# ectucker1/voxel-raytracing

Hardware: AMD Instinct MI355X
Metric: Mrays/sec at 1080p treehouse.vox; achieved HBM GB/s vs MI355X peak (higher is better)
Workload: dtype f32; 1 GPU; synthetic:treehouse(seed=2) 256^3 stand-in for treehouse.vox, 1920x1080, primary rays only (BASELINE configs[1]); 128 frame(s)/step (128 per GPU, consecutive poses, one K1 launch per step), 16-row strips over 1 GPU(s); traversal=AUTO, bytes_out_per_px=37, device=AMD Radeon Graphics (gfx950:sramecc+:xnack-)

## Files before the change

voxel-raytracing_amd/csrc/vrt_api.hip:

```cpp
#include <cstdio>
#include <cstdlib>
#include <cstring>

#include "image_io.h"
#include "vox_reader.h"
#include "vrt_host.h"

using namespace vrt;

static thread_local std::string g_err;

int vrt::fail(int code, const std::string& msg) { g_err = msg; return code; }

struct OptName { const char* name; const char* env; int DevOptions::*field; };
static const OptName kOptNames[] = {
    {"tile_tags", "VRT_TILE_TAGS", &DevOptions::tile_tags}, {"box_rect", "VRT_BOX_RECT", &DevOptions::box_rect},
    {"xcd_regions", "VRT_XCD_REGIONS", &DevOptions::xcd_regions}, {"fast_loop", "VRT_FAST_LOOP", &DevOptions::fast_loop},
    {"no_bounce_kernel", "VRT_NO_BOUNCE_KERNEL", &DevOptions::no_bounce_kernel}, {"sky_fast", "VRT_SKY_FAST", &DevOptions::sky_fast},
    {"sky_span", "VRT_SKY_SPAN", &DevOptions::sky_span},
    {"packed_bounces", "VRT_PACKED_BOUNCES", &DevOptions::packed_bounces}, {"ao_batch", "VRT_AO_BATCH", &DevOptions::ao_batch}, {"tags_async", "VRT_TAGS_ASYNC", &DevOptions::tags_async},
    {"hit_table", "VRT_HIT_TABLE", &DevOptions::hit_table},
    {"thresh_runs", "VRT_THRESH_RUNS", &DevOptions::thresh_runs}, {"segment_budget", "VRT_SEGMENT_BUDGET", &DevOptions::segment_budget}, {"denoise_th16", "VRT_DENOISE_TH", &DevOptions::denoise_th16}, {"denoise_packed", "VRT_DENOISE_PACKED", &DevOptions::denoise_packed},
    {"denoise_pair", "VRT_DENOISE_PAIR", &DevOptions::denoise_pair}, {"denoise_p0", "VRT_DENOISE_P0", &DevOptions::denoise_p0}, {"denoise_pair_wgs", "VRT_DENOISE_PAIR_WGS", &DevOptions::denoise_pair_wgs},
    {"denoise_verified", "VRT_DENOISE_VERIFIED", &DevOptions::denoise_verified}, {"denoise_guard_div8", "VRT_DENOISE_GUARD_DIV8", &DevOptions::denoise_guard_div8},
    {"denoise_count", "VRT_DENOISE_COUNT", &DevOptions::denoise_count},
    {"open_cells", "VRT_OPEN_CELLS", &DevOptions::open_cells}, {"df_prefetch", "VRT_DF_PREFETCH", &DevOptions::df_prefetch},
    {"df_own", "VRT_DF_OWN", &DevOptions::df_own},
};

extern "C" {

const char* vrt_last_error(void) { return g_err.c_str(); }

int vrt_ctx_create(int device, vrt_ctx** out)
{
    if (!out) return fail(VRT_ERR_INVALID, "vrt_ctx_create: out is NULL");
    int n = 0;
    hipError_t e = hipGetDeviceCount(&n);
    if (e != hipSuccess || n <= 0)
        return fail(VRT_ERR_NO_DEVICE, std::string("no HIP device available (") + hipGetErrorString(e) +
                                           "); this library has no CPU fallback");
    if (device < 0 || device >= n) return fail(VRT_ERR_INVALID, "vrt_ctx_create: device index out of range");
    HIPCHK(hipSetDevice(device));
    vrt_ctx* c = new vrt_ctx();
    c->device = device;
    for (const OptName& o : kOptNames) {
        const char* e = getenv(o.env);
        if (e && e[0] >= '0' && e[0] <= '9') c->opt.*(o.field) = atoi(e);
    }
// ... 460 lines not shown
        c->tile_tags[b].reset(); c->tile_tags_words[b] = 0;
        HIPCHK(c->tile_tags[b].alloc((words + 3) * sizeof(uint32_t)));
        HIPCHK(hipMemsetAsync(c->tile_tags[b].get(), 0, (words + 3) * sizeof(uint32_t), c->stream));
        HIPCHK(hipStreamSynchronize(c->stream));
        c->tile_tags_words[b] = words;
        c->tag_read_valid[b] = false;
    }
    if (++c->tile_gen == 0u) {
        HIPCHK(hipStreamSynchronize(c->stream));
        if (c->tag_stream) HIPCHK(hipStreamSynchronize(c->tag_stream));
        for (int q = 0; q < 2; q++)
            if (c->tile_tags[q]) HIPCHK(hipMemsetAsync(c->tile_tags[q].get(), 0, c->tile_tags_words[q] * sizeof(uint32_t), c->stream));
        HIPCHK(hipStreamSynchronize(c->stream));
        c->tile_gen = 1u;
    }
    p.tile_tags = c->tile_tags[b].get(); p.tile_gen = c->tile_gen;
    if (p.fused_shade == 1 && p.table) {
        const size_t bytes = (size_t)vrt::verdict_pitch((uint32_t)(p.tiles_x * (p.tile_w / 8))) * (size_t)(p.tiles_y_local * (p.tile_h / 8)) * (size_t)n;
        if (c->verdict_bytes[b] < bytes) {
            HIPCHK(hipStreamSynchronize(c->stream));
            if (c->tag_stream) HIPCHK(hipStreamSynchronize(c->tag_stream));
            c->verdicts[b].reset(); c->verdict_bytes[b] = 0;
            HIPCHK(c->verdicts[b].alloc(bytes));
            c->verdict_bytes[b] = bytes;
        }
        p.verdicts = c->verdicts[b].get();
    }
    if (!tags) {
        std::vector<uint32_t> ones((size_t)n, c->tile_gen);
        HIPCHK(hipMemcpyAsync(c->tile_tags[b].get(), ones.data(), (size_t)n * 4, hipMemcpyHostToDevice, c->stream));
        HIPCHK(launch_block_verdicts(p, c->stream));
        return VRT_OK;
    }
    p.cells = s->cells.get(); p.n_cells = s->n_cells; p.cell_size = s->bricks ? 8u : 4u;
    const bool async = c->opt.tags_async >= 2 || (c->opt.tags_async != 0 && hipStreamQuery(c->stream) == hipErrorNotReady);
    if (!async) {
        HIPCHK(launch_tile_tags(p, c->stream));
        HIPCHK(launch_block_verdicts(p, c->stream));
        return VRT_OK;
    }
    if (!c->tag_stream) {
        HIPCHK(hipStreamCreateWithFlags(&c->tag_stream, hipStreamNonBlocking));
        for (int q = 0; q < 2; q++) {
            HIPCHK(hipEventCreateWithFlags(&c->tag_done[q], hipEventDisableTiming));
            HIPCHK(hipEventCreateWithFlags(&c->tag_read[q], hipEventDisableTiming));
        }
        HIPCHK(hipEventRecord(c->tag_read[b], c->stream));
        HIPCHK(hipStreamWaitEvent(c->tag_stream, c->tag_read[b], 0));
    }
    if (c->tag_read_valid[b]) HIPCHK(hipStreamWaitEvent(c->tag_stream, c->tag_read[b], 0));
    if (tab >= 0) HIPCHK(hipStreamWaitEvent(c->tag_stream, c->tab_uploaded[tab], 0));
    HIPCHK(launch_tile_tags(p, c->tag_stream));
    HIPCHK(launch_block_verdicts(p, c->tag_stream));
    HIPCHK(hipEventRecord(c->tag_done[b], c->tag_stream));
    HIPCHK(hipStreamWaitEvent(c->stream, c->tag_done[b], 0));
    return VRT_OK;
}

static int render_frames(vrt_ctx* c, const vrt_scene* s, int n, const vrt_push* pushes, const vrt_settings* st,
                         const vrt_frame* frames, const vrt_shard* shards, int per_frame)
{
    const Launch l = {n, pushes, st, frames, shards, per_frame, pushes[0].screen_size[0], pushes[0].screen_size[1]};
    int rc = launch_args(c, s, l);
    if (rc != VRT_OK) return rc;
    const bool counts = count_planes(l);
    const uint8_t* count_fields = nullptr;
    if (counts && !s->bricks && s->open_cells) {
// ... 240 lines not shown
```

voxel-raytracing_amd/csrc/vrt_api_edit.hip:

```cpp
#include <cstddef>
#include <cstring>

#include "vrt_host.h"
#include "vrt_brush_launch.h"
#include "vrt_flood_launch.h"
#include "vrt_voxelize_launch.h"
#include "vrt_morph_launch.h"
#include "vrt_components_launch.h"

using namespace vrt;

static_assert(VRT_BRUSH_BOX == VRT_BRUSH_SHAPE_BOX && VRT_BRUSH_ELLIPSOID == VRT_BRUSH_SHAPE_ELLIPSOID && VRT_BRUSH_CAPSULE == VRT_BRUSH_SHAPE_CAPSULE,
              "include/vrt.h and csrc/vrt_brush.h number the shapes differently");
static_assert(VRT_BRUSH_SET == VRT_BRUSH_MODE_SET && VRT_BRUSH_PAINT == VRT_BRUSH_MODE_PAINT && VRT_BRUSH_ADD == VRT_BRUSH_MODE_ADD &&
              VRT_BRUSH_REPLACE == VRT_BRUSH_MODE_REPLACE, "include/vrt.h and csrc/vrt_brush.h number the modes differently");
static_assert(VRT_FLOOD_SAME == VRT_FLOOD_MATCH_SAME && VRT_FLOOD_SOLID == VRT_FLOOD_MATCH_SOLID && VRT_FLOOD_FACES == VRT_FLOOD_CONN_FACES &&
              VRT_FLOOD_CORNERS == VRT_FLOOD_CONN_CORNERS && VRT_FLOOD_MEASURE == VRT_FLOOD_FLAG_MEASURE,
              "include/vrt.h and csrc/vrt_flood.h number the predicates, connectivities or flags differently");
static_assert(VRT_VOXELIZE_SURFACE == VRT_VOXELIZE_FILL_SURFACE && VRT_VOXELIZE_SOLID == VRT_VOXELIZE_FILL_SOLID,
              "include/vrt.h and csrc/vrt_voxelize.h number the fills differently");
static_assert(VRT_MORPH_DILATE == VRT_MORPH_OP_DILATE && VRT_MORPH_ERODE == VRT_MORPH_OP_ERODE && VRT_MORPH_OPEN == VRT_MORPH_OP_OPEN &&
              VRT_MORPH_CLOSE == VRT_MORPH_OP_CLOSE && VRT_MORPH_HOLLOW == VRT_MORPH_OP_HOLLOW && VRT_MORPH_FACES == VRT_MORPH_CONN_FACES &&
              VRT_MORPH_CORNERS == VRT_MORPH_CONN_CORNERS && VRT_MORPH_BORDER_SOLID == VRT_MORPH_FLAG_BORDER_SOLID && VRT_MORPH_MEASURE == VRT_MORPH_FLAG_MEASURE,
              "include/vrt.h and csrc/vrt_morph.h number the operations, connectivities or flags differently");
// ... 57 lines not shown
    b.nb[0] = d.W / 8; b.nb[1] = d.H / 8; b.nb[2] = d.D / 8;
    b.n = (size_t)b.nb[0] * b.nb[1] * b.nb[2];
    b.npad = ((size_t)b.nb[0] + 2u) * ((size_t)b.nb[1] + 2u) * ((size_t)b.nb[2] + 2u);
    b.cstride = (size_t)d.bcoarse_stride;
    return b;
}

uint64_t brick_scene_bytes(const vrt_scene* s)
{
    const BrickDims b = brick_dims(s);
    return b.npad * 8ull + (uint64_t)s->bcap * 512ull * 9ull + 256 * sizeof(vrt_material) + (uint64_t)s->cells_room * 4ull +
           b.npad * 4ull + b.n + 8ull * b.cstride + s->scratch_bytes();
}

void brick_cell_add(vrt_scene* s, uint32_t slot, uint32_t pc)
{
    s->cell_pos[slot] = (uint32_t)s->hcells.size();
    s->hcells.push_back(brick_cell_code(pc, s->d.vol.pbx, s->d.vol.pby));
    s->cell_slot.push_back(slot);
}

void brick_cell_remove(vrt_scene* s, uint32_t slot)
{
    const uint32_t pos = s->cell_pos[slot], last = (uint32_t)s->hcells.size() - 1u;
    s->hcells[pos] = s->hcells[last]; s->cell_slot[pos] = s->cell_slot[last];
    s->cell_pos[s->cell_slot[pos]] = pos;
    s->hcells.pop_back(); s->cell_slot.pop_back();
    s->cell_pos[slot] = kNoBrick;
}

hipError_t brick_upload_cells(vrt_scene* s)
{
    const size_t n = s->hcells.size();
    s->n_cells = 0; s->cells_ok = false;
    if (n > kMaxCells || n > s->cells_room) return hipSuccess;
    if (n) { const hipError_t e = hipMemcpy(s->cells.get(), s->hcells.data(), n * 4, hipMemcpyHostToDevice); if (e != hipSuccess) return e; }
    s->n_cells = (uint32_t)n; s->cells_ok = true;
    return hipSuccess;
}

hipError_t brick_build_coarse(vrt_ctx* c, vrt_scene* s, uint8_t* tmp0, uint8_t* tmp1, bool pack)
{
    const BrickDims b = brick_dims(s);
    hipError_t e = launch_build_df(s->bocc.get(), b.nb[0], b.nb[1], b.nb[2], s->bcoarse.get(), b.cstride, tmp0, tmp1, c->stream, VRT_BRICK_EDIT_CAP);
    if (e == hipSuccess && s->open_cells) e = launch_open_cells(s->bocc.get(), b.nb[0], b.nb[1], b.nb[2], s->bcoarse.get(), b.cstride, tmp0, tmp1, c->stream, 0x80);
    if (e == hipSuccess && pack) e = launch_brick_pack(s->bgrid.get(), s->bcoarse.get(), b.cstride, b.npad, s->bentry.get(), c->stream);
    return e;
}

int brick_scene_edit(vrt_ctx* c, vrt_scene* s, const EditBox& box, const EditIds& src, const std::string& name)
{
    const VolumeView& d = s->d.vol;
    const BrickDims bd = brick_dims(s);
    BrickEdit e;
    e.nbx = bd.nb[0]; e.nby = bd.nb[1]; e.nbz = bd.nb[2]; e.pbx = d.pbx; e.pby = d.pby;
    EditSpan f[3];
    size_t nT = 1, nF = 1, nbox = 1;
    for (int a = 0; a < 3; a++) {
        e.lo[a] = box.lo[a]; e.hi[a] = box.hi[a];
        const EditSpan t = brick_span_t(box.lo[a], box.hi[a]);
        e.t_lo[a] = t.lo; e.t_n[a] = t.hi - t.lo;
        f[a] = brick_span_f(t, bd.nb[a]);
        nT *= (size_t)e.t_n[a]; nF *= (size_t)(f[a].hi - f[a].lo); nbox *= (size_t)(box.hi[a] - box.lo[a]);
    }
    const bool rule = brick_edit_in_place(e.nbx, e.nby, e.nbz, box.lo, box.hi);
    const bool ids = src.boxed();
    const size_t ids_room = ids ? round256(nbox) : 0, t_room = round256(nT * 4);
    const size_t list_max = rule ? nF : ((size_t)s->n_occ + nT < (size_t)s->bcap ? (size_t)s->n_occ + nT : (size_t)s->bcap);
    const size_t list_room = round256(list_max * 8);
    const size_t coarse_room = rule ? bedit_coarse_scratch_bytes(e, bd.cstride, s->open_cells) : 2 * round256(bd.n);
// ... 799 lines not shown
```

voxel-raytracing_amd/csrc/vrt_api_scene.hip:

```cpp
#include <atomic>
#include <cstdio>
#include <cstring>
#include <memory>

#include "image_io.h"
#include "vox_reader.h"
#include "vox_writer.h"
#include "vrt_host.h"
#define VRT_SCENE_READ_LAUNCHERS
#include "vrt_scene_read.h"

using namespace vrt;

static std::atomic<uint64_t> g_shade_gen{0};

extern "C" {

void vrt_scene_free(vrt_ctx* c, vrt_scene* s)
{
    if (!s) return;
    if (c) { hipSetDevice(c->device); hipStreamSynchronize(c->stream); }
    delete s;
}

// ... 55 lines not shown
    return rc == VRT_OK ? vrt_scene_set_blue_noise(c, s, grey, 1, 1) : rc;
}

void vrt::drop_count_fields(vrt_scene* s)
{
    if (!s->df_counts) return;
    s->df_counts_raw.reset(); s->df_counts = nullptr;
    s->bytes -= s->df_bytes;
}

hipError_t vrt::build_fields(vrt_ctx* c, const vrt_scene* s, uint8_t* dst, bool open)
{
    const VolumeView& d = s->d.vol;
    const size_t nvox = (size_t)d.W * (size_t)d.H * (size_t)d.D, ndf = df_field_bytes(d.W, d.H, d.D);
    hipError_t e = hipMemsetAsync(dst, 0, s->df_bytes, c->stream);
    if (e != hipSuccess) return e;
    if (d.df_fast) {
        if ((e = hipMemsetAsync(dst + 9 * ndf, 0xFF, 1, c->stream)) != hipSuccess) return e;
        if ((e = launch_pad_vox(s->vox.get(), d.W, d.H, d.D, dst + 8 * ndf, c->stream)) != hipSuccess) return e;
    }
    DevBuf<uint8_t> tmp0, tmp1;
    if ((e = tmp0.alloc(nvox)) != hipSuccess) return e;
    e = tmp1.alloc(nvox);
    if (e == hipSuccess) e = launch_build_df(s->vox.get(), d.W, d.H, d.D, dst, ndf, tmp0.get(), tmp1.get(), c->stream);
    if (e == hipSuccess && open) e = launch_open_cells(s->vox.get(), d.W, d.H, d.D, dst, ndf, tmp0.get(), tmp1.get(), c->stream);
    const hipError_t sync = hipStreamSynchronize(c->stream);
    return e != hipSuccess ? e : sync;
}

hipError_t vrt::build_cell_list(vrt_ctx* c, vrt_scene* s)
{
    const VolumeView& d = s->d.vol;
    if (s->cells) { s->cells.reset(); s->bytes -= (uint64_t)s->n_cells * 4; }
    s->n_cells = 0; s->cells_ok = false;
    if (d.n1x > 1024 || d.n1y > 1024 || d.n1z > 1024) return hipSuccess;
    const size_t n2 = (size_t)d.n2x * d.n2y * d.n2z;
    std::vector<uint64_t> h2(n2);
    hipError_t e = hipMemcpyAsync(h2.data(), s->occ2.get(), n2 * 8, hipMemcpyDeviceToHost, c->stream);
    if (e == hipSuccess) e = hipStreamSynchronize(c->stream);
    if (e != hipSuccess) return e;
    std::vector<uint32_t> cells;
    for (size_t w = 0; w < n2; w++) {
        uint64_t bits = h2[w];
        if (!bits) continue;
        const uint32_t wx = (uint32_t)(w % (size_t)d.n2x), wy = (uint32_t)((w / (size_t)d.n2x) % (size_t)d.n2y), wz = (uint32_t)(w / ((size_t)d.n2x * d.n2y));
        for (uint32_t b = 0; b < 64; b++)
            if ((bits >> b) & 1ull) cells.push_back((wx * 4u + (b & 3u)) | ((wy * 4u + ((b >> 2) & 3u)) << 10) | ((wz * 4u + (b >> 4)) << 20));
    }
    if (cells.size() > kMaxCells) return hipSuccess;
    if (!cells.empty()) {
        if ((e = s->cells.alloc(cells.size() * 4)) != hipSuccess) return e;
        if ((e = hipMemcpy(s->cells.get(), cells.data(), cells.size() * 4, hipMemcpyHostToDevice)) != hipSuccess) return e;
        s->bytes += cells.size() * 4;
    }
    s->n_cells = (uint32_t)cells.size();
    s->cells_ok = true;
    return hipSuccess;
}

int vrt::fields_for_counts(vrt_ctx* c, const vrt_scene* cs, const uint8_t** out)
{
    vrt_scene* s = const_cast<vrt_scene*>(cs);
    std::lock_guard<std::mutex> lock(s->lazy);
    if (!s->open_cells) { *out = s->df; return VRT_OK; }
    if (!s->df_counts) {
        size_t free_b = 0, total_b = 0;
        if (hipMemGetInfo(&free_b, &total_b) == hipSuccess && (uint64_t)s->df_bytes + 2ull * (uint64_t)s->d.vol.W * s->d.vol.H * s->d.vol.D > (uint64_t)free_b)
            return fail(VRT_ERR_UNSUPPORTED, "vrt_render_geometry: the count planes (steps_primary, steps_total) need a second set of clearance fields (" +
                        std::to_string((uint64_t)s->df_bytes) + " bytes), which does not fit the device memory that is free");
        DevBuf<uint8_t> p;
        HIPCHK(p.alloc(s->df_bytes + 2 * s->df_guard));
        hipError_t e = hipMemsetAsync(p.get(), 0, s->df_bytes + 2 * s->df_guard, c->stream);
        if (e == hipSuccess) e = build_fields(c, s, p.get() + s->df_guard, false);
        if (e != hipSuccess) return fail(VRT_ERR_HIP, std::string("building the count planes' clearance fields: ") + hipGetErrorString(e));
        s->df_counts_raw = std::move(p); s->df_counts = s->df_counts_raw.get() + s->df_guard;
        s->bytes += s->df_bytes;
    }
    *out = s->df_counts;
    return VRT_OK;
}

uint32_t vrt::brick_cell_code(uint32_t pc, int pbx, int pby)
{
    return (uint32_t)(pc % (uint32_t)pbx - 1u) | ((uint32_t)((pc / (uint32_t)pbx) % (uint32_t)pby - 1u) << 10) | ((uint32_t)(pc / ((uint32_t)pbx * (uint32_t)pby) - 1u) << 20);
}

extern "C" {

// ... 101 lines not shown
        DevBuf<uint32_t> grid_dev, coord_dev;
        DevBuf<uint8_t> occ_dev, tmp0_dev, tmp1_dev;
        HIPCHK(s->bgrid.alloc(npad * 4));
        HIPCHK(s->bcoarse.alloc(8 * cstride));
        HIPCHK(s->bpool.alloc(pool_bytes ? pool_bytes : 1));
        HIPCHK(s->bfine.alloc(fine_bytes ? fine_bytes : 1));
        HIPCHK(s->palette.alloc(256 * sizeof(vrt_material)));
        HIPCHK(grid_dev.alloc(nb * 4));
        HIPCHK(coord_dev.alloc((size_t)(n_bricks ? n_bricks : 1) * 4));
        HIPCHK(occ_dev.alloc(nb));
        HIPCHK(tmp0_dev.alloc(nb));
        HIPCHK(tmp1_dev.alloc(nb));
        uint8_t *occ = occ_dev.get(), *tmp0 = tmp0_dev.get(), *tmp1 = tmp1_dev.get();
        s->bytes = npad * 4ull + 8ull * cstride + pool_bytes + fine_bytes + 256 * sizeof(vrt_material);
        HIPCHK(hipMemsetAsync(s->bgrid.get(), 0xFF, npad * 4, c->stream));
        HIPCHK(hipMemsetAsync(s->bcoarse.get(), 0, 8 * cstride, c->stream));
        HIPCHK(hipMemcpyAsync(grid_dev.get(), grid, nb * 4, hipMemcpyHostToDevice, c->stream));
        if (n_bricks) {
            HIPCHK(hipMemcpyAsync(coord_dev.get(), coord.data(), (size_t)n_bricks * 4, hipMemcpyHostToDevice, c->stream));
            HIPCHK(hipMemcpyAsync(s->bpool.get(), pool, pool_bytes, hipMemcpyHostToDevice, c->stream));
        }
        HIPCHK(hipMemcpyAsync(s->palette.get(), palette, 256 * sizeof(vrt_material), hipMemcpyHostToDevice, c->stream));
        HIPCHK(launch_brick_grid(grid_dev.get(), (int)nbx, (int)nby, (int)nbz, s->bgrid.get(), occ, c->stream));
        HIPCHK(launch_build_df(occ, (int)nbx, (int)nby, (int)nbz, s->bcoarse.get(), cstride, tmp0, tmp1, c->stream, VRT_BRICK_EDIT_CAP));
        {
            s->open_cells = c->opt.open_cells != 0;
            if (s->open_cells) HIPCHK(launch_open_cells(occ, (int)nbx, (int)nby, (int)nbz, s->bcoarse.get(), cstride, tmp0, tmp1, c->stream, 0x80));
            d.brick_open = s->open_cells ? 1u : 0u;
            d.df_own = c->opt.df_own ? 1u : 0u;
        }
        if (n_bricks <= kMaxCells) {
            std::vector<uint32_t> cells(n_bricks);
            for (uint32_t i = 0; i < n_bricks; i++) cells[i] = brick_cell_code(coord[i], d.pbx, d.pby);
            if (n_bricks) {
                HIPCHK(s->cells.alloc((size_t)n_bricks * 4));
                HIPCHK(hipMemcpy(s->cells.get(), cells.data(), (size_t)n_bricks * 4, hipMemcpyHostToDevice));
                s->bytes += (uint64_t)n_bricks * 4;
            }
            s->n_cells = n_bricks; s->cells_ok = true;
        }
        HIPCHK(launch_brick_fine(s->bgrid.get(), (int)pbx, (int)pby, coord_dev.get(), n_bricks, s->bpool.get(), s->bfine.get(), c->stream));
        HIPCHK(s->bentry.alloc(npad * 8));
        HIPCHK(launch_brick_pack(s->bgrid.get(), s->bcoarse.get(), cstride, npad, s->bentry.get(), c->stream));
        HIPCHK(hipStreamSynchronize(c->stream));
        s->bgrid.reset(); s->bcoarse.reset();
        s->bytes = npad * 8ull + pool_bytes + fine_bytes + 256 * sizeof(vrt_material) + (uint64_t)n_bricks * 4;
        s->bcap = n_bricks;
    }
    d.bgrid = nullptr; d.bcoarse = nullptr; d.bcoarse_stride = cstride; d.bpool = s->bpool.get(); d.bfine = s->bfine.get(); d.bentry = s->bentry.get();
    s->d.palette = s->palette.get();
    const int rc = default_textures(c, s);
    if (rc != VRT_OK) return rc;
    *out = hold.release();
    return VRT_OK;
}

int vrt_scene_trim(vrt_ctx* c, vrt_scene* s)
{
    if (!c || !s) return fail(VRT_ERR_INVALID, "vrt_scene_trim: NULL argument");
    HIPCHK(hipSetDevice(c->device));
    HIPCHK(hipDeviceSynchronize());
    std::lock_guard<std::mutex> lock(s->lazy);
    drop_count_fields(s);
    s->drop_scratch();
    return VRT_OK;
}
// ... 275 lines not shown
```

voxel-raytracing_amd/csrc/vrt_device.hip:

```cpp
#include "vrt_shade.h"
#include "vrt_frame_slot.h"

namespace vrt {


template <int TRAV, bool OCC_LDS, int MODE, bool TABLE, int MAP>
__global__ __launch_bounds__(256) __attribute__((amdgpu_waves_per_eu(7, 8))) void k_primary(const GeomParams P)
{
    extern __shared__ __attribute__((aligned(16))) uint64_t lds_occ[];
    TileMap M = P.map;
    const uint64_t t_begin = (M.flags & 2u) ? wall_clock64() : 0ull;
    int x0, y0, yp0, ty, tx;
    uint32_t frame;
    if (!block_to_tile<MAP>(M, frame, ty, tx)) return;
    const int wave = __builtin_amdgcn_readfirstlane((int)(threadIdx.x >> 6));
    const uint32_t tile_gen = P.tile_gen;
    constexpr bool kVerdict = MODE == 1 && TABLE;
    constexpr bool kOneFetch = MODE == 1 && !kVerdict;
    typedef uint32_t span_words __attribute__((ext_vector_type(4), aligned(4)));
    span_words st;
    uint32_t tag_all = 0u, own = 0u, tag = 0u, vword = 0u, role = 0u;
    bool span_w = false, wide = false;
    if constexpr (kVerdict) {
        const uint32_t sh = (uint32_t)M.tile >> 4;
// ... 425 lines not shown
{
    hipLaunchKernelGGL(k_hit_colors, dim3(64), dim3(256), 0, s, p, table);
    return hipGetLastError();
}

template <bool TABLE>
__global__ __launch_bounds__(256) void k_tile_tags(const GeomParams P)
{
    const uint32_t frame = blockIdx.y;
    RayGenConsts g;
    float cam[3], U[3];
    int shard_rank;
    uint32_t box;
    SlotOf<TABLE>::head(P, frame, g, U, shard_rank, box);
    if (box == 0xFF00FF00u) return;
    { const f3 cp = SlotOf<TABLE>::cam_pos(P, frame); cam[0] = cp.x; cam[1] = cp.y; cam[2] = cp.z; }
    const uint32_t ci = blockIdx.x * 256u + threadIdx.x;
    if (ci >= P.n_cells) return;
    const uint32_t cell = P.cells[ci];
    const uint32_t cs = P.cell_size;
    const float ext = (float)cs + 2.0f;
    const float lo[3] = {(float)((cell & 1023u) * cs) - 1.0f, (float)(((cell >> 10) & 1023u) * cs) - 1.0f, (float)((cell >> 20) * cs) - 1.0f};
    uint32_t* tags = P.tile_tags + (size_t)frame * P.tags_per_frame;
    TagCam tc;
    tc.U[0] = U[0]; tc.U[1] = U[1]; tc.U[2] = U[2];
    tc.V[0] = g.planeV.x; tc.V[1] = g.planeV.y; tc.V[2] = g.planeV.z;
    tc.C[0] = g.cd.x + g.jx; tc.C[1] = g.cd.y + g.jy; tc.C[2] = g.cd.z;
    tc.cam[0] = cam[0]; tc.cam[1] = cam[1]; tc.cam[2] = cam[2];
    tc.W = g.W; tc.H = g.H;
    if (P.sh.nranks > 1) {
        const int rows = P.sh.strip_rows, total = ((int)g.H + rows - 1) / rows;
        if (shard_rank + P.sh.nranks >= total && tag_band_cull(tc, lo, ext, (float)(shard_rank * rows), (float)(shard_rank * rows + rows))) return;
    }
    float x0, x1, y0, y1, ex, ey;
    const int st = tag_project(tc, lo, ext, x0, x1, y0, y1, ex, ey);
    bool all = (st & 1) != 0;
    const float m = VRT_TAG_MARGIN_PX;
    if (!all) {
        const float gx = fmaxf(m, ex + 0.5f), gy = fmaxf(m, ey + 0.5f);
        if (x1 + gx < 0.0f || y1 + gy < 0.0f || x0 - gx > g.W || y0 - gy > g.H) return;
        if (st & 2) all = true;
    }
    int tx0 = (int)floorf(fmaxf(x0 - m, 0.0f) * 0.125f), tx1 = (int)floorf(fminf(x1 + m, g.W - 1.0f) * 0.125f);
    int ty0 = (int)floorf(fmaxf(y0 - m, 0.0f) * 0.125f), ty1 = (int)floorf(fminf(y1 + m, g.H - 1.0f) * 0.125f);
    if (!all && (tx1 - tx0 + 1) * (ty1 - ty0 + 1) > 1024) all = true;
    if (all) { tags[P.tags_per_frame - 1u] = P.tile_gen; return; }
    const int nranks = P.sh.nranks, rows8 = P.sh.strip_rows >> 3, k = P.tile_h >> 3, T = P.tiles_y_local;
    if (nranks <= 1) {
        for (int ty = ty0; ty <= ty1; ty++) {
            const int tyl = ty / k;
            if (tyl >= T) continue;
            const uint32_t row = (uint32_t)((T - 1 - tyl) * k + (ty - tyl * k));
            for (int tx = tx0; tx <= tx1; tx++) tags[row * P.tags_x + (uint32_t)tx] = P.tile_gen;
        }
        return;
    }
    const int s0 = ty0 / rows8, s1 = ty1 / rows8;
    int s = s0 + ((shard_rank - s0 % nranks) + nranks) % nranks;
    for (; s <= s1; s += nranks) {
        const int a = ty0 > s * rows8 ? ty0 : s * rows8, b = ty1 < (s + 1) * rows8 - 1 ? ty1 : (s + 1) * rows8 - 1;
        for (int ty = a; ty <= b; ty++) {
            const int local = (s / nranks) * rows8 + (ty - s * rows8);
            const int tyl = local / k;
            if (tyl >= T) continue;
            const uint32_t row = (uint32_t)((T - 1 - tyl) * k + (local - tyl * k));
            for (int tx = tx0; tx <= tx1; tx++) tags[row * P.tags_x + (uint32_t)tx] = P.tile_gen;
        }
    }
}

hipError_t launch_tile_tags(const GeomParams& p, hipStream_t s)
{
    if (p.n_cells == 0u) return hipSuccess;
    dim3 grid((p.n_cells + 255u) / 256u, (unsigned)p.n_frames), block(256);
    if (p.table) hipLaunchKernelGGL(k_tile_tags<true>, grid, block, 0, s, p);
    else         hipLaunchKernelGGL(k_tile_tags<false>, grid, block, 0, s, p);
    return hipGetLastError();
}

// ... 71 lines not shown
```

voxel-raytracing_amd/csrc/vrt_host.h:

```cpp
#pragma once
#include <mutex>
#include <string>
#include <vector>

#include "vrt_internal.h"

namespace vrt {

int fail(int code, const std::string& msg);

#define HIPCHK(expr)                                                                              \
    do {                                                                                          \
        hipError_t e_ = (expr);                                                                   \
        if (e_ != hipSuccess)                                                                     \
            return ::vrt::fail(VRT_ERR_HIP, std::string(#expr) + ": " + hipGetErrorString(e_));   \
    } while (0)

inline int ceil_div(int a, int b) { return (a + b - 1) / b; }

template <class T>
class DevBuf {
public:
    DevBuf() = default;
    DevBuf(DevBuf&& o) noexcept : p_(o.p_), bytes_(o.bytes_) { o.p_ = nullptr; o.bytes_ = 0; }
// ... 15 lines not shown
    }
    void reset() { if (p_) hipFree(p_); p_ = nullptr; bytes_ = 0; }
    T* get() const { return p_; }
    size_t bytes() const { return bytes_; }
    explicit operator bool() const { return p_ != nullptr; }

private:
    T* p_ = nullptr;
    size_t bytes_ = 0;
};

struct Scratch {
    DevBuf<uint8_t> buf;
    size_t bytes = 0;
    uint8_t* get() const { return buf.get(); }
    void drop(uint64_t& total) { if (buf) { buf.reset(); total -= bytes; } bytes = 0; }
    hipError_t room(size_t need, uint64_t& total)
    {
        if (need <= bytes) return hipSuccess;
        drop(total);
        const hipError_t e = buf.alloc(need);
        if (e == hipSuccess) { bytes = need; total += need; }
        return e;
    }
};

const size_t kMaxCells = (size_t)4u << 20;
inline size_t round256(size_t n) { return (n + 255u) & ~(size_t)255u; }

}

struct DevOptions {
    int tile_tags = 1;
    int box_rect = 1;
    int xcd_regions = 0;
    int fast_loop = 1;
    int no_bounce_kernel = 1;
    int packed_bounces = 1;
    int tags_async = 0;
    int ao_batch = 1;
    int sky_fast = 1;
    int sky_span = 1;
    int thresh_runs = 1;
    int segment_budget = 1;
    int hit_table = 1;
    int denoise_th16 = 0;
    int denoise_packed = 1;
    int denoise_pair = 1;
    int denoise_p0 = 1;
    int denoise_pair_wgs = 0;
    int denoise_verified = 1;
    int denoise_guard_div8 = 0;
    int denoise_count = 0;
    int open_cells = 1;
    int df_prefetch = 1;
    int df_own = 1;
};

struct vrt_ctx {
    int device = 0;
    DevOptions opt;
    hipStream_t stream = nullptr;
    bool own_stream = true;
    bool timing = true;
    hipEvent_t ev_geo0 = nullptr, ev_prim1 = nullptr, ev_geo1 = nullptr, ev_den0 = nullptr, ev_den1 = nullptr;
    bool have_geo = false, have_den = false;
// ... 14 lines not shown
    size_t tile_tags_words[2] = {0, 0};
    vrt::DevBuf<uint8_t> verdicts[2];
    size_t verdict_bytes[2] = {0, 0};
    uint32_t tile_gen = 0;
    int tag_flip = 0;
    hipStream_t tag_stream = nullptr;
    hipEvent_t tag_done[2] = {nullptr, nullptr};
    hipEvent_t tag_read[2] = {nullptr, nullptr};
    bool tag_read_valid[2] = {false, false};
    vrt::DevBuf<uint32_t> hit_colors;
    uint64_t hit_scene_gen = 0;
    vrt::DevBuf<uint32_t> den_counts;
    int den_last_passes = 0;
    vrt_settings hit_settings{};
    vrt::DevBuf<float> pano_dev;
    float* pano_host = nullptr;
    size_t pano_floats = 0;
    hipEvent_t pano_done = nullptr;
    bool pano_busy = false;
    vrt::DevBuf<uint8_t> brush_rec;
};

struct vrt_scene {
    vrt::DevScene d{};
    vrt::DevBuf<uint8_t> vox;
    vrt::DevBuf<uint64_t> occ1, occ2, occ3;
    vrt::DevBuf<uint8_t> df_raw;
    uint8_t* df = nullptr;
    vrt::DevBuf<uint8_t> df_counts_raw;
    uint8_t* df_counts = nullptr;
    bool metallic_voxels = true;
    vrt::DevBuf<uint32_t> cells;
    uint32_t n_cells = 0;
    bool cells_ok = false;
    bool open_cells = false;
    size_t df_bytes = 0;
    size_t df_guard = 0;
    std::mutex lazy;
    vrt::DevBuf<vrt_material> palette;
    vrt::DevBuf<float> sky;
    vrt::DevBuf<uint8_t> noise;
    vrt::DevBuf<float> sky_normals;
    vrt::DevBuf<uint32_t> sky8;
    uint32_t occ2_bytes = 0, occ3_bytes = 0;
    vrt::DevBuf<uint32_t> bgrid; vrt::DevBuf<uint8_t> bcoarse, bpool, bfine;
    vrt::DevBuf<uint64_t> bentry;
    bool bricks = false;
    uint32_t bcap = 0;
    bool reserved = false;
    vrt::DevBuf<uint8_t> bocc;
    uint32_t n_occ = 0;
    size_t cells_room = 0;
    std::vector<uint32_t> hgrid;
    std::vector<uint32_t> slot_pc;
    std::vector<uint32_t> free_slots;
    std::vector<uint32_t> hcells, cell_slot, cell_pos;
    uint64_t bytes = 0;
    bool metal[256] = {};
    vrt::Scratch edit_scratch;
    vrt::Scratch flood_scratch;
    uint32_t flood_rounds = 0;
    vrt::Scratch voxelize_scratch;
    uint32_t voxelize_item_rows = 0, voxelize_items = 0;
    vrt::Scratch morph_scratch;
    vrt::Scratch comp_scratch, comp_table;
    uint64_t edit_gen = 0, comp_gen = 0;
// ... 39 lines not shown
```

voxel-raytracing_amd/csrc/vrt_tags.h:

```cpp
#pragma once

#include "vrt_spec.h"

namespace vrt {

#define VRT_TAG_MARGIN_PX 2.0f
#define VRT_TAG_ERR_MAX_PX 1.5f

struct TagCam {
    float U[3], V[3], C[3], cam[3];
    float W, H;
};

#if defined(__HIP_DEVICE_COMPILE__)
__device__ __forceinline__ float tag_rcp(float x) { return __builtin_amdgcn_rcpf(x); }
#else
static thread_local int g_tag_rcp_ulps = 0;
inline float tag_rcp(float x)
{
    union { float f; int32_t i; } c; c.f = (float)(1.0 / (double)x);
    c.i += (c.f > 0.0f ? 1 : -1) * g_tag_rcp_ulps;
    return c.f;
}
#endif

VRT_HD int tag_project(const TagCam& k, const float lo[3], float ext, float& x0, float& x1, float& y0, float& y1, float& ex, float& ey)
{
    const float* U = k.U; const float* V = k.V; const float* C = k.C;
    const float c0[3] = {V[1] * C[2] - V[2] * C[1], V[2] * C[0] - V[0] * C[2], V[0] * C[1] - V[1] * C[0]};
    const float c1[3] = {C[1] * U[2] - C[2] * U[1], C[2] * U[0] - C[0] * U[2], C[0] * U[1] - C[1] * U[0]};
    const float c2[3] = {U[1] * V[2] - U[2] * V[1], U[2] * V[0] - U[0] * V[2], U[0] * V[1] - U[1] * V[0]};
    const float m0[3] = {fabsf(V[1] * C[2]) + fabsf(V[2] * C[1]), fabsf(V[2] * C[0]) + fabsf(V[0] * C[2]), fabsf(V[0] * C[1]) + fabsf(V[1] * C[0])};
    const float m1[3] = {fabsf(C[1] * U[2]) + fabsf(C[2] * U[1]), fabsf(C[2] * U[0]) + fabsf(C[0] * U[2]), fabsf(C[0] * U[1]) + fabsf(C[1] * U[0])};
    const float m2[3] = {fabsf(U[1] * V[2]) + fabsf(U[2] * V[1]), fabsf(U[2] * V[0]) + fabsf(U[0] * V[2]), fabsf(U[0] * V[1]) + fabsf(U[1] * V[0])};
// ... 3 lines not shown
    const float p0[3] = {lo[0] - k.cam[0], lo[1] - k.cam[1], lo[2] - k.cam[2]};
    const float A0 = p0[0] * c0[0] + p0[1] * c0[1] + p0[2] * c0[2], B0 = p0[0] * c1[0] + p0[1] * c1[1] + p0[2] * c1[2];
    const float L0 = p0[0] * c2[0] + p0[1] * c2[1] + p0[2] * c2[2];
    const float pa[3] = {fabsf(p0[0]) + ext, fabsf(p0[1]) + ext, fabsf(p0[2]) + ext};
    const float Q0 = pa[0] * m0[0] + pa[1] * m0[1] + pa[2] * m0[2], Q1 = pa[0] * m1[0] + pa[1] * m1[1] + pa[2] * m1[2];
    const float Q2 = pa[0] * m2[0] + pa[1] * m2[1] + pa[2] * m2[2];
    const float hw = 0.5f * k.W, hh = 0.5f * k.H;
    const float sgn = det < 0.0f ? -1.0f : 1.0f;
    x0 = 1e30f; x1 = -1e30f; y0 = 1e30f; y1 = -1e30f;
    float lmin = 1e30f;
#if defined(__HIP_DEVICE_COMPILE__)
#pragma unroll
#endif
    for (int c = 0; c < 8; c++) {
        const float dx = (c & 1) ? ext : 0.0f, dy = (c & 2) ? ext : 0.0f, dz = (c & 4) ? ext : 0.0f;
        const float An = A0 + (dx * c0[0] + dy * c0[1] + dz * c0[2]), Bn = B0 + (dx * c1[0] + dy * c1[1] + dz * c1[2]);
        const float Ln = L0 + (dx * c2[0] + dy * c2[1] + dz * c2[2]);
        lmin = fminf(lmin, Ln * sgn);
        const float rl = tag_rcp(Ln);
        const float fx = An * rl * hw + hw, fy = Bn * rl * hh + hh;
        x0 = fminf(x0, fx); x1 = fmaxf(x1, fx); y0 = fminf(y0, fy); y1 = fmaxf(y1, fy);
    }
    const float u = 5.9604645e-8f;
    if (!(lmin > 16.0f * u * Q2)) all = true;
    if (!(x0 == x0) || !(x1 == x1) || !(y0 == y0) || !(y1 == y1)) all = true;
    const float amax = fmaxf(fabsf(x0 - hw), fabsf(x1 - hw)) * tag_rcp(hw), bmax = fmaxf(fabsf(y0 - hh), fabsf(y1 - hh)) * tag_rcp(hh);
    const float rL = tag_rcp(lmin);
    ex = 8.0f * u * hw * (Q0 + amax * Q2) * rL + 10.0f * u * hw * (amax + 1.0f);
    ey = 8.0f * u * hh * (Q1 + bmax * Q2) * rL + 10.0f * u * hh * (bmax + 1.0f);
    const bool loose = !(ex <= VRT_TAG_ERR_MAX_PX) || !(ey <= VRT_TAG_ERR_MAX_PX);
    return (all ? 1 : 0) | (loose ? 2 : 0);
}

VRT_HD bool tag_band_cull(const TagCam& k, const float lo[3], float ext, float ylo, float yhi)
{
    const float* U = k.U; const float* V = k.V; const float* C = k.C;
    const float c0[3] = {V[1] * C[2] - V[2] * C[1], V[2] * C[0] - V[0] * C[2], V[0] * C[1] - V[1] * C[0]};
    const float c1[3] = {C[1] * U[2] - C[2] * U[1], C[2] * U[0] - C[0] * U[2], C[0] * U[1] - C[1] * U[0]};
    const float c2[3] = {U[1] * V[2] - U[2] * V[1], U[2] * V[0] - U[0] * V[2], U[0] * V[1] - U[1] * V[0]};
    const float m0[3] = {fabsf(V[1] * C[2]) + fabsf(V[2] * C[1]), fabsf(V[2] * C[0]) + fabsf(V[0] * C[2]), fabsf(V[0] * C[1]) + fabsf(V[1] * C[0])};
    const float m1[3] = {fabsf(C[1] * U[2]) + fabsf(C[2] * U[1]), fabsf(C[2] * U[0]) + fabsf(C[0] * U[2]), fabsf(C[0] * U[1]) + fabsf(C[1] * U[0])};
    const float m2[3] = {fabsf(U[1] * V[2]) + fabsf(U[2] * V[1]), fabsf(U[2] * V[0]) + fabsf(U[0] * V[2]), fabsf(U[0] * V[1]) + fabsf(U[1] * V[0])};
    const float det = U[0] * c0[0] + U[1] * c0[1] + U[2] * c0[2];
    const float mdet = fabsf(U[0]) * m0[0] + fabsf(U[1]) * m0[1] + fabsf(U[2]) * m0[2];
    if (!(fabsf(det) > 1e-5f * mdet)) return false;
    const float sgn = det < 0.0f ? -1.0f : 1.0f;
    const float p0[3] = {lo[0] - k.cam[0], lo[1] - k.cam[1], lo[2] - k.cam[2]};
    const float B0 = (p0[0] * c1[0] + p0[1] * c1[1] + p0[2] * c1[2]) * sgn, L0 = (p0[0] * c2[0] + p0[1] * c2[1] + p0[2] * c2[2]) * sgn;
    const float pa[3] = {fabsf(p0[0]) + ext, fabsf(p0[1]) + ext, fabsf(p0[2]) + ext};
    const float Q1 = pa[0] * m1[0] + pa[1] * m1[1] + pa[2] * m1[2], Q2 = pa[0] * m2[0] + pa[1] * m2[1] + pa[2] * m2[2];
    const float u = 5.9604645e-8f;
    const float l0 = c2[0] * sgn * ext, l1 = c2[1] * sgn * ext, l2 = c2[2] * sgn * ext;
    const float lmin = L0 + (fminf(l0, 0.0f) + fminf(l1, 0.0f) + fminf(l2, 0.0f));
    if (!(lmin > 16.0f * u * Q2)) return false;
    const float hh = 0.5f * k.H, rh = tag_rcp(hh);
    const float m = VRT_TAG_MARGIN_PX;
    const float tlo = ((ylo - m) - hh) * rh, thi = ((yhi + m) - hh) * rh;
    const float b0 = c1[0] * sgn * ext, b1 = c1[1] * sgn * ext, b2 = c1[2] * sgn * ext;
    {
        const float f0 = b0 - tlo * l0, f1 = b1 - tlo * l1, f2 = b2 - tlo * l2;
        const float fmax = (B0 - tlo * L0) + (fmaxf(f0, 0.0f) + fmaxf(f1, 0.0f) + fmaxf(f2, 0.0f));
        const float E = 16.0f * u * (Q1 + (fabsf(tlo) + 1.0f) * Q2);
        if (fmax < -E) return true;
    }
    {
        const float f0 = b0 - thi * l0, f1 = b1 - thi * l1, f2 = b2 - thi * l2;
// ... 9 lines not shown
```

Before: 106,200 Mrays/s.

## Restrict tile tagging to surface cells by sorting interior cells last

```diff
diff --git a/voxel-raytracing_amd/csrc/vrt_api.hip b/voxel-raytracing_amd/csrc/vrt_api.hip
--- a/voxel-raytracing_amd/csrc/vrt_api.hip
+++ b/voxel-raytracing_amd/csrc/vrt_api.hip
@@ -14,7 +14,7 @@
 
 struct OptName { const char* name; const char* env; int DevOptions::*field; };
 static const OptName kOptNames[] = {
-    {"tile_tags", "VRT_TILE_TAGS", &DevOptions::tile_tags}, {"box_rect", "VRT_BOX_RECT", &DevOptions::box_rect},
+    {"tile_tags", "VRT_TILE_TAGS", &DevOptions::tile_tags}, {"tag_surface", "VRT_TAG_SURFACE", &DevOptions::tag_surface}, {"box_rect", "VRT_BOX_RECT", &DevOptions::box_rect},
     {"xcd_regions", "VRT_XCD_REGIONS", &DevOptions::xcd_regions}, {"fast_loop", "VRT_FAST_LOOP", &DevOptions::fast_loop},
     {"no_bounce_kernel", "VRT_NO_BOUNCE_KERNEL", &DevOptions::no_bounce_kernel}, {"sky_fast", "VRT_SKY_FAST", &DevOptions::sky_fast},
     {"sky_span", "VRT_SKY_SPAN", &DevOptions::sky_span},
@@ -541,7 +541,7 @@
         HIPCHK(launch_block_verdicts(p, c->stream));
         return VRT_OK;
     }
-    p.cells = s->cells.get(); p.n_cells = s->n_cells; p.cell_size = s->bricks ? 8u : 4u;
+    p.cells = s->cells.get(); p.n_cells = c->opt.tag_surface ? s->n_tag_cells : s->n_cells; p.cell_size = s->bricks ? 8u : 4u;
     const bool async = c->opt.tags_async >= 2 || (c->opt.tags_async != 0 && hipStreamQuery(c->stream) == hipErrorNotReady);
     if (!async) {
         HIPCHK(launch_tile_tags(p, c->stream));
diff --git a/voxel-raytracing_amd/csrc/vrt_api_edit.hip b/voxel-raytracing_amd/csrc/vrt_api_edit.hip
--- a/voxel-raytracing_amd/csrc/vrt_api_edit.hip
+++ b/voxel-raytracing_amd/csrc/vrt_api_edit.hip
@@ -113,10 +113,19 @@
 hipError_t brick_upload_cells(vrt_scene* s)
 {
     const size_t n = s->hcells.size();
-    s->n_cells = 0; s->cells_ok = false;
+    s->n_cells = 0; s->n_tag_cells = 0; s->cells_ok = false;
     if (n > kMaxCells || n > s->cells_room) return hipSuccess;
-    if (n) { const hipError_t e = hipMemcpy(s->cells.get(), s->hcells.data(), n * 4, hipMemcpyHostToDevice); if (e != hipSuccess) return e; }
-    s->n_cells = (uint32_t)n; s->cells_ok = true;
+    std::vector<uint32_t> dev(s->hcells), back(n);
+    const int pbx = s->d.vol.pbx, pby = s->d.vol.pby;
+    const auto occupied = [&](int x, int y, int z) {
+        const uint32_t g = s->hgrid[(size_t)(x + 1) + ((size_t)(y + 1) + (size_t)(z + 1) * (size_t)pby) * (size_t)pbx];
+        return g != 0u && g != 0xFFFFFFFFu;
+    };
+    const uint32_t n_surface = tag_surface_first(dev.data(), (uint32_t)n, back.data(), [&](uint32_t cell) {
+        return tag_cell_is_surface(occupied, (int)(cell & 1023u), (int)((cell >> 10) & 1023u), (int)(cell >> 20));
+    });
+    if (n) { const hipError_t e = hipMemcpy(s->cells.get(), dev.data(), n * 4, hipMemcpyHostToDevice); if (e != hipSuccess) return e; }
+    s->n_cells = (uint32_t)n; s->n_tag_cells = n_surface; s->cells_ok = true;
     return hipSuccess;
 }
 
diff --git a/voxel-raytracing_amd/csrc/vrt_api_scene.hip b/voxel-raytracing_amd/csrc/vrt_api_scene.hip
--- a/voxel-raytracing_amd/csrc/vrt_api_scene.hip
+++ b/voxel-raytracing_amd/csrc/vrt_api_scene.hip
@@ -111,7 +111,7 @@
 {
     const VolumeView& d = s->d.vol;
     if (s->cells) { s->cells.reset(); s->bytes -= (uint64_t)s->n_cells * 4; }
-    s->n_cells = 0; s->cells_ok = false;
+    s->n_cells = 0; s->n_tag_cells = 0; s->cells_ok = false;
     if (d.n1x > 1024 || d.n1y > 1024 || d.n1z > 1024) return hipSuccess;
     const size_t n2 = (size_t)d.n2x * d.n2y * d.n2z;
     std::vector<uint64_t> h2(n2);
@@ -127,12 +127,23 @@
             if ((bits >> b) & 1ull) cells.push_back((wx * 4u + (b & 3u)) | ((wy * 4u + ((b >> 2) & 3u)) << 10) | ((wz * 4u + (b >> 4)) << 20));
     }
     if (cells.size() > kMaxCells) return hipSuccess;
+    uint32_t n_surface = 0;
+    if (!cells.empty()) {
+        std::vector<uint64_t> inner(n2), tmp(n2);
+        tag_interior_words(h2.data(), d.n2x, d.n2y, d.n2z, inner.data(), tmp.data());
+        std::vector<uint32_t> back(cells.size());
+        n_surface = tag_surface_first(cells.data(), (uint32_t)cells.size(), back.data(), [&](uint32_t cell) {
+            const uint32_t x = cell & 1023u, y = (cell >> 10) & 1023u, z = cell >> 20;
+            const size_t w = (size_t)(x >> 2) + (size_t)d.n2x * ((size_t)(y >> 2) + (size_t)d.n2y * (size_t)(z >> 2));
+            return !((inner[w] >> ((x & 3u) | ((y & 3u) << 2) | ((z & 3u) << 4))) & 1ull);
+        });
+    }
     if (!cells.empty()) {
         if ((e = s->cells.alloc(cells.size() * 4)) != hipSuccess) return e;
         if ((e = hipMemcpy(s->cells.get(), cells.data(), cells.size() * 4, hipMemcpyHostToDevice)) != hipSuccess) return e;
         s->bytes += cells.size() * 4;
     }
-    s->n_cells = (uint32_t)cells.size();
+    s->n_cells = (uint32_t)cells.size(); s->n_tag_cells = n_surface;
     s->cells_ok = true;
     return hipSuccess;
 }
@@ -300,6 +311,13 @@
         if (n_bricks <= kMaxCells) {
             std::vector<uint32_t> cells(n_bricks);
             for (uint32_t i = 0; i < n_bricks; i++) cells[i] = brick_cell_code(coord[i], d.pbx, d.pby);
+            std::vector<uint32_t> back(n_bricks);
+            const auto occupied = [&](int x, int y, int z) {
+                return x >= 0 && y >= 0 && z >= 0 && x < (int)nbx && y < (int)nby && z < (int)nbz && grid[(size_t)x + (size_t)nbx * ((size_t)y + (size_t)nby * (size_t)z)] != 0u;
+            };
+            s->n_tag_cells = tag_surface_first(cells.data(), n_bricks, back.data(), [&](uint32_t cell) {
+                return tag_cell_is_surface(occupied, (int)(cell & 1023u), (int)((cell >> 10) & 1023u), (int)(cell >> 20));
+            });
             if (n_bricks) {
                 HIPCHK(s->cells.alloc((size_t)n_bricks * 4));
                 HIPCHK(hipMemcpy(s->cells.get(), cells.data(), (size_t)n_bricks * 4, hipMemcpyHostToDevice));
diff --git a/voxel-raytracing_amd/csrc/vrt_device.hip b/voxel-raytracing_amd/csrc/vrt_device.hip
--- a/voxel-raytracing_amd/csrc/vrt_device.hip
+++ b/voxel-raytracing_amd/csrc/vrt_device.hip
@@ -481,19 +481,10 @@
         const int rows = P.sh.strip_rows, total = ((int)g.H + rows - 1) / rows;
         if (shard_rank + P.sh.nranks >= total && tag_band_cull(tc, lo, ext, (float)(shard_rank * rows), (float)(shard_rank * rows + rows))) return;
     }
-    float x0, x1, y0, y1, ex, ey;
-    const int st = tag_project(tc, lo, ext, x0, x1, y0, y1, ex, ey);
-    bool all = (st & 1) != 0;
-    const float m = VRT_TAG_MARGIN_PX;
-    if (!all) {
-        const float gx = fmaxf(m, ex + 0.5f), gy = fmaxf(m, ey + 0.5f);
-        if (x1 + gx < 0.0f || y1 + gy < 0.0f || x0 - gx > g.W || y0 - gy > g.H) return;
-        if (st & 2) all = true;
-    }
-    int tx0 = (int)floorf(fmaxf(x0 - m, 0.0f) * 0.125f), tx1 = (int)floorf(fminf(x1 + m, g.W - 1.0f) * 0.125f);
-    int ty0 = (int)floorf(fmaxf(y0 - m, 0.0f) * 0.125f), ty1 = (int)floorf(fminf(y1 + m, g.H - 1.0f) * 0.125f);
-    if (!all && (tx1 - tx0 + 1) * (ty1 - ty0 + 1) > 1024) all = true;
-    if (all) { tags[P.tags_per_frame - 1u] = P.tile_gen; return; }
+    int tx0, tx1, ty0, ty1;
+    const int what = tag_cell_blocks(tc, lo, ext, tx0, tx1, ty0, ty1);
+    if (what == 0) return;
+    if (what == 2) { tags[P.tags_per_frame - 1u] = P.tile_gen; return; }
     const int nranks = P.sh.nranks, rows8 = P.sh.strip_rows >> 3, k = P.tile_h >> 3, T = P.tiles_y_local;
     if (nranks <= 1) {
         for (int ty = ty0; ty <= ty1; ty++) {
diff --git a/voxel-raytracing_amd/csrc/vrt_host.h b/voxel-raytracing_amd/csrc/vrt_host.h
--- a/voxel-raytracing_amd/csrc/vrt_host.h
+++ b/voxel-raytracing_amd/csrc/vrt_host.h
@@ -71,6 +71,7 @@
 
 struct DevOptions {
     int tile_tags = 1;
+    int tag_surface = 1;
     int box_rect = 1;
     int xcd_regions = 0;
     int fast_loop = 1;
@@ -151,6 +152,7 @@
     bool metallic_voxels = true;
     vrt::DevBuf<uint32_t> cells;
     uint32_t n_cells = 0;
+    uint32_t n_tag_cells = 0;
     bool cells_ok = false;
     bool open_cells = false;
     size_t df_bytes = 0;
diff --git a/voxel-raytracing_amd/csrc/vrt_tags.h b/voxel-raytracing_amd/csrc/vrt_tags.h
--- a/voxel-raytracing_amd/csrc/vrt_tags.h
+++ b/voxel-raytracing_amd/csrc/vrt_tags.h
@@ -1,5 +1,6 @@
 #pragma once
 
+#include <stddef.h>
 #include "vrt_spec.h"
 
 namespace vrt {
@@ -69,6 +70,60 @@
     return (all ? 1 : 0) | (loose ? 2 : 0);
 }
 
+VRT_HD int tag_cell_blocks(const TagCam& k, const float lo[3], float ext, int& tx0, int& tx1, int& ty0, int& ty1)
+{
+    float x0, x1, y0, y1, ex, ey;
+    const int st = tag_project(k, lo, ext, x0, x1, y0, y1, ex, ey);
+    const float m = VRT_TAG_MARGIN_PX;
+    if (st & 1) return 2;
+    const float gx = fmaxf(m, ex + 0.5f), gy = fmaxf(m, ey + 0.5f);
+    if (x1 + gx < 0.0f || y1 + gy < 0.0f || x0 - gx > k.W || y0 - gy > k.H) return 0;
+    if (st & 2) return 2;
+    tx0 = (int)floorf(fmaxf(x0 - m, 0.0f) * 0.125f); tx1 = (int)floorf(fminf(x1 + m, k.W - 1.0f) * 0.125f);
+    ty0 = (int)floorf(fmaxf(y0 - m, 0.0f) * 0.125f); ty1 = (int)floorf(fminf(y1 + m, k.H - 1.0f) * 0.125f);
+    return (tx1 - tx0 + 1) * (ty1 - ty0 + 1) > 1024 ? 2 : 1;
+}
+
+
+inline void tag_interior_words(const uint64_t* occ, int nx, int ny, int nz, uint64_t* out, uint64_t* tmp)
+{
+    const size_t sy = (size_t)nx, sz = (size_t)nx * (size_t)ny;
+    for (int z = 0; z < nz; z++) for (int y = 0; y < ny; y++) for (int x = 0; x < nx; x++) {
+        const size_t i = (size_t)x + sy * (size_t)y + sz * (size_t)z;
+        const uint64_t w = occ[i], l = x > 0 ? occ[i - 1] : 0ull, r = x + 1 < nx ? occ[i + 1] : 0ull;
+        out[i] = w & (((w << 1) & 0xEEEEEEEEEEEEEEEEull) | ((l >> 3) & 0x1111111111111111ull))
+                   & (((w >> 1) & 0x7777777777777777ull) | ((r << 3) & 0x8888888888888888ull));
+    }
+    for (int z = 0; z < nz; z++) for (int y = 0; y < ny; y++) for (int x = 0; x < nx; x++) {
+        const size_t i = (size_t)x + sy * (size_t)y + sz * (size_t)z;
+        const uint64_t w = out[i], l = y > 0 ? out[i - sy] : 0ull, r = y + 1 < ny ? out[i + sy] : 0ull;
+        tmp[i] = w & (((w << 4) & 0xFFF0FFF0FFF0FFF0ull) | ((l >> 12) & 0x000F000F000F000Full))
+                   & (((w >> 4) & 0x0FFF0FFF0FFF0FFFull) | ((r << 12) & 0xF000F000F000F000ull));
+    }
+    for (int z = 0; z < nz; z++) for (int y = 0; y < ny; y++) for (int x = 0; x < nx; x++) {
+        const size_t i = (size_t)x + sy * (size_t)y + sz * (size_t)z;
+        const uint64_t w = tmp[i], l = z > 0 ? tmp[i - sz] : 0ull, r = z + 1 < nz ? tmp[i + sz] : 0ull;
+        out[i] = w & ((w << 16) | (l >> 48)) & ((w >> 16) | (r << 48));
+    }
+}
+
+template <class Occ>
+inline bool tag_cell_is_surface(const Occ& occupied, int x, int y, int z)
+{
+    for (int dz = -1; dz <= 1; dz++) for (int dy = -1; dy <= 1; dy++) for (int dx = -1; dx <= 1; dx++)
+        if (!occupied(x + dx, y + dy, z + dz)) return true;
+    return false;
+}
+
+template <class IsSurface>
+inline uint32_t tag_surface_first(uint32_t* cells, uint32_t n, uint32_t* tmp, const IsSurface& is_surface)
+{
+    uint32_t ns = 0, ni = 0;
+    for (uint32_t i = 0; i < n; i++) { if (is_surface(cells[i])) cells[ns++] = cells[i]; else tmp[ni++] = cells[i]; }
+    for (uint32_t i = 0; i < ni; i++) cells[ns + i] = tmp[i];
+    return ns;
+}
+
 VRT_HD bool tag_band_cull(const TagCam& k, const float lo[3], float ext, float ylo, float yhi)
 {
     const float* U = k.U; const float* V = k.V; const float* C = k.C;
```

New measurement: 106,400 Mrays/s, median of 6. About the same (+0.2%).
